# YXHXianYu/RVCP-Real-Time-Path-Tracer

Measured on AMD Instinct MI355X. Metric: Msamples/sec (pixels*SPP/s) + frame ms, Cornell Box 1024^2 SPP=30, higher is better.
Workload: dtype f32

## Files before the change

### rvcp-real-time-path-tracer_amd/csrc/embed_src.py

```python
#!/usr/bin/env python3
import hashlib
import sys

NAMES = ["kJitSrcKernels", "kJitSrcInternal", "kJitSrcAbi", "kJitSrcSqrt", "kJitSrcTonemap"]
DELIM = "RVCPSRC"


def build_id(out, srcs):
    h = hashlib.sha256()
    for path in srcs:
        data = open(path, "rb").read()
        h.update(path.encode() + b"\0" + str(len(data)).encode() + b"\0" + data)
    with open(out, "w") as f:
        f.write("// generated by embed_src.py --build-id; do not edit\n#pragma once\n"
                f'static const char kRvcpSourceHash[] = "{h.hexdigest()[:16]}";\n')


def main():
    if sys.argv[1] == "--build-id":
        return build_id(sys.argv[2], sys.argv[3:])
    out, srcs = sys.argv[1], sys.argv[2:]
    parts = ["// generated by embed_src.py from " + " ".join(srcs) + "; do not edit", "#pragma once"]
    for name, path in zip(NAMES, srcs):
        text = open(path).read()
        assert ")" + DELIM + '"' not in text
        parts.append(f'static const char {name}[] = R"{DELIM}(' + text + f'){DELIM}";')
    with open(out, "w") as f:
        f.write("\n".join(parts) + "\n")


if __name__ == "__main__":
    main()
```

### rvcp-real-time-path-tracer_amd/csrc/rvcp_jit.cpp

```cpp
#include <hip/hip_runtime.h>

#include <dlfcn.h>
#include <sys/stat.h>
#include <unistd.h>

#include <algorithm>
#include <atomic>
#include <cerrno>
#include <cmath>
#include <cstdint>
#include <cstdio>
#include <cstdlib>
#include <cstring>
#include <list>
#include <memory>
#include <mutex>
#include <map>
#include <string>
#include <vector>

#include "rvcp_internal.h"
#include "rvcp_jit.h"
#include "build/rvcp_jit_src.h"

// ... 789 lines not shown
    e = std::getenv("RVCP_DEBUG_SPEC_EAGER");
    if (e && *e == '1') opts |= kScanEagerSplit;
#endif
    return opts;
}

std::vector<std::string> jit_options(const JitCompile &cc);

std::string jit_sampling_tag(int sampling)
{
    return sampling == RVCP_SAMPLING_UNIFORM ? std::string()
                                             : "// +sampling " + std::to_string(sampling) + "\n";
}

std::string jit_spp_map_tag(bool spp_map)
{
    return spp_map ? std::string("// +spp_map\n") : std::string();
}

namespace {

uint64_t fnv1a(const std::string &s)
{
    uint64_t h = 1469598103934665603ull;
    for (unsigned char c : s) {
        h ^= c;
        h *= 1099511628211ull;
    }
    return h;
}

struct CacheEntry {
    int device;
    uint64_t hash;
    std::string scan;
    std::shared_ptr<JitKernels> kernels;
};
std::mutex g_mu;
std::list<CacheEntry> g_cache;
constexpr size_t kCacheEntries = 16;

constexpr char kCoMagic[8] = {'R', 'V', 'C', 'P', 'C', 'O', '0', '1'};
std::string g_cache_dir;
bool g_cache_dir_set = false;
std::atomic<uint64_t> g_disk_loads{0}, g_disk_compiles{0}, g_disk_rejects{0};

std::string default_cache_dir()
{
    const char *x = std::getenv("XDG_CACHE_HOME");
    if (x && *x == '/') return std::string(x) + "/rvcp-mi355x";
    const char *h = std::getenv("HOME");
    if (h && *h == '/') return std::string(h) + "/.cache/rvcp-mi355x";
    return std::string();
}

std::string cache_dir()
{
    if (!g_cache_dir_set) {
        g_cache_dir = default_cache_dir();
        g_cache_dir_set = true;
    }
    return g_cache_dir;
}

bool make_dirs(const std::string &dir)
{
    if (dir.empty()) return false;
    for (size_t i = 1; i <= dir.size(); i++) {
        if (i == dir.size() || dir[i] == '/') {
            const std::string p = dir.substr(0, i);
            if (::mkdir(p.c_str(), 0700) != 0 && errno != EEXIST) return false;
        }
    }
    struct stat st;
    return ::stat(dir.c_str(), &st) == 0 && S_ISDIR(st.st_mode);
}

std::string code_key(const std::string &scan, const std::vector<std::string> &opts)
{
    int maj = -1, mnr = -1;
    if (rtc().version) (void)rtc().version(&maj, &mnr);
    std::string k = "rvcp code object\nhiprtc " + std::to_string(maj) + "." + std::to_string(mnr) + "\n";
    for (const std::string &o : opts) k += o + "\n";
    for (const char *src : {kJitSrcKernels, kJitSrcInternal, kJitSrcAbi, kJitSrcSqrt, kJitSrcTonemap}) {
        const std::string s(src);
        k += "src " + std::to_string(s.size()) + " " + std::to_string(fnv1a(s)) + "\n";
    }
    return k + scan;
}

std::string hex64(uint64_t v)
{
    char b[17];
    std::snprintf(b, sizeof(b), "%016llx", (unsigned long long)v);
    return b;
}

uint64_t fnv1a_bytes(const char *p, size_t n)
{
    uint64_t h = 1469598103934665603ull;
    for (size_t i = 0; i < n; i++) {
        h ^= (unsigned char)p[i];
        h *= 1099511628211ull;
    }
    return h;
}

int disk_read(const std::string &dir, const std::string &key, std::vector<char> &code)
{
    const std::string path = dir + "/" + hex64(fnv1a(key)) + ".rvcpco";
    std::FILE *f = std::fopen(path.c_str(), "rb");
    if (!f) return 0;
    std::vector<char> buf;
    char tmp[1 << 16];
    size_t got;
    while ((got = std::fread(tmp, 1, sizeof(tmp), f)) > 0) buf.insert(buf.end(), tmp, tmp + got);
    std::fclose(f);
    uint64_t hdr[4];
    if (buf.size() < 8 + sizeof(hdr) || std::memcmp(buf.data(), kCoMagic, 8) != 0) return -1;
    std::memcpy(hdr, buf.data() + 8, sizeof(hdr));
    const size_t off = 8 + sizeof(hdr);
    if (hdr[0] != key.size() || hdr[1] == 0 || buf.size() - off < hdr[0] ||
        buf.size() - off - hdr[0] != hdr[1] ||
        hdr[3] != fnv1a(key) || std::memcmp(buf.data() + off, key.data(), key.size()) != 0)
        return -1;
    const char *c = buf.data() + off + hdr[0];
    if (fnv1a_bytes(c, hdr[1]) != hdr[2] || hdr[1] < 4 || std::memcmp(c, "\x7f" "ELF", 4) != 0)
        return -1;
    code.assign(c, c + hdr[1]);
    return 1;
}

void disk_write(const std::string &dir, const std::string &key, const std::vector<char> &code)
{
    if (!make_dirs(dir)) return;
    static std::atomic<unsigned> seq{0};
    const std::string path = dir + "/" + hex64(fnv1a(key)) + ".rvcpco";
    const std::string tmp = path + ".tmp." + std::to_string((long)::getpid()) + "." + std::to_string(seq++);
    std::FILE *f = std::fopen(tmp.c_str(), "wb");
    if (!f) return;
    const uint64_t hdr[4] = {key.size(), code.size(), fnv1a_bytes(code.data(), code.size()), fnv1a(key)};
    bool ok = std::fwrite(kCoMagic, 1, 8, f) == 8 && std::fwrite(hdr, 1, sizeof(hdr), f) == sizeof(hdr) &&
              std::fwrite(key.data(), 1, key.size(), f) == key.size() &&
              std::fwrite(code.data(), 1, code.size(), f) == code.size();
    ok = (std::fclose(f) == 0) && ok;
    if (!ok || std::rename(tmp.c_str(), path.c_str()) != 0) std::remove(tmp.c_str());
}

}

int jit_cached_code(const std::string &scan, std::vector<char> &code, std::string &err,
                    const JitCompile &cc, bool *from_disk, bool force_compile)
{
    *from_disk = false;
    const std::string dir = cache_dir();
    std::string key;
    if (!dir.empty()) {
        key = code_key(scan, jit_options(cc));
        if (force_compile) {
            g_disk_rejects++;
        } else {
            const int r = disk_read(dir, key, code);
            if (r == 1) {
                g_disk_loads++;
                *from_disk = true;
                return 0;
            }
            if (r < 0) g_disk_rejects++;
        }
    }
    if (jit_compile_code(scan, code, err, cc) != 0) return -1;
    g_disk_compiles++;
    if (!dir.empty()) disk_write(dir, key, code);
    return 0;
}

JitKernels::~JitKernels()
{
    if (module) {
        int cur = -1;
        (void)hipGetDevice(&cur);
        (void)hipSetDevice(device);
        (void)hipModuleUnload(module);
        if (cur >= 0) (void)hipSetDevice(cur);
    }
}

std::vector<std::string> jit_options(const JitCompile &cc)
{
    std::vector<std::string> opts = {"--offload-arch=gfx950", "-O3", "-std=c++17",
                                     "-ffp-contract=off", "-fhip-fp32-correctly-rounded-divide-sqrt",
                                     "-fno-fast-math", "-fno-slp-vectorize", "-DRVCP_JIT",
                                     "-DRVCP_SPEC_SCAN=\"rvcp_spec_scan.inc\""};
    if (cc.legacy) opts.push_back("-DRVCP_JIT_LEGACY");
    if (cc.bvh) opts.push_back("-DRVCP_JIT_BVH");
    if (cc.sampling != RVCP_SAMPLING_UNIFORM)
        opts.push_back("-DRVCP_SAMPLING=" + std::to_string(cc.sampling));
    if (cc.spp_map) opts.push_back("-DRVCP_SPP_MAP=1");
#ifdef RVCP_TIMELINE
    opts.push_back("-DRVCP_TIMELINE");
#endif
    if (cc.legacy && cc.legacy_waves > 0)
        opts.push_back("-DRVCP_LEGACY_MIN_WAVES=" + std::to_string(cc.legacy_waves));
    if (cc.legacy && cc.lds_scene) opts.push_back("-DRVCP_LEGACY_LDS_SCENE");
    for (const std::string &x : jit_extra_flags()) opts.push_back(x);
    return opts;
}

int jit_compile_code(const std::string &scan, std::vector<char> &code, std::string &err,
                     const JitCompile &cc)
{
    const RtcApi &api = rtc();
    if (!api.ok) {
        err = api.why;
        return -1;
    }
    const char *hdr_src[] = {kJitSrcInternal, kJitSrcAbi, kJitSrcSqrt, kJitSrcTonemap, scan.c_str()};
    const char *hdr_name[] = {"rvcp_internal.h", "../../include/rvcp.h", "rvcp_sqrt.h", "rvcp_tonemap.h",
                              "rvcp_spec_scan.inc"};
    rtc_program prog = nullptr;
    if (api.create(&prog, kJitSrcKernels, "rvcp_kernels.hip", 5, hdr_src, hdr_name) != 0) {
        err = "hiprtcCreateProgram failed";
        return -1;
    }
    const std::vector<std::string> opt_s = jit_options(cc);
    std::vector<const char *> opts;
    for (const std::string &x : opt_s) opts.push_back(x.c_str());
    const int rc = api.compile(prog, (int)opts.size(), opts.data());
    if (rc != 0) {
        size_t ls = 0;
        api.log_size(prog, &ls);
        std::string log(ls, '\0');
        if (ls) api.log(prog, &log[0]);
        err = "hipRTC compile failed: " + log.substr(0, 4000);
        api.destroy(&prog);
        return -1;
    }
    size_t cs = 0;
    api.code_size(prog, &cs);
    code.assign(cs, 0);
    if (cs) api.code(prog, code.data());
    api.destroy(&prog);
    return cs ? 0 : -1;
}

std::string jit_module_source(const TriRecord *tri, uint32_t n, const JitSpec &spec, JitCompile &cc)
{
    cc = JitCompile{};
    cc.legacy = spec.legacy;
    cc.lds_scene = spec.legacy && spec.lds_fits;
#ifndef RVCP_SPHERELESS_LEGACY_WAVES
#define RVCP_SPHERELESS_LEGACY_WAVES 6
#endif
    cc.legacy_waves = spec.legacy && spec.sphereless ? RVCP_SPHERELESS_LEGACY_WAVES : cc.lds_scene ? 5 : 0;
#ifdef RVCP_DEBUG_KNOBS
    if (const char *e = std::getenv("RVCP_JIT_LEGACY_WAVES")) cc.legacy_waves = std::atoi(e);
#endif
    cc.bvh = spec.bvh;
    cc.sampling = spec.sampling;
    cc.spp_map = spec.spp_map;
    std::string key_flags;
    for (const std::string &x : jit_extra_flags()) key_flags += " " + x;
    return jit_scan_source(tri, n, jit_scan_opts()) +
        (spec.legacy || spec.bvh ? std::string() : jit_groups_source(tri, n, spec.lum_mask, jit_scan_opts())) +
        (spec.legacy ? "// +legacy " + std::to_string(cc.legacy_waves) + (cc.lds_scene ? " lds" : "") + "\n"
#ifndef RVCP_NO_SPHERE_LITERALS
                      + jit_sphere_source(spec.spheres, spec.n_spheres)
#endif
                      + (cc.lds_scene ? jit_legacy_lds_source(n, spec.n_spheres, spec.n_materials) : std::string())
                : std::string()) +
        (key_flags.empty() ? std::string() : "// +flags" + key_flags + "\n") +
        (spec.bvh ? "// +bvh\n" : "") +
        jit_sampling_tag(spec.sampling) + jit_spp_map_tag(spec.spp_map);
}

std::shared_ptr<JitKernels> jit_path_kernels(int device, const TriRecord *tri, uint32_t n,
                                             const JitSpec &spec, std::string &err)
{
    JitCompile cc;
    const std::string scan = jit_module_source(tri, n, spec, cc);
    const bool legacy = spec.legacy, bvh = spec.bvh;
    const uint64_t h = fnv1a(scan);
    std::lock_guard<std::mutex> lock(g_mu);
    for (auto it = g_cache.begin(); it != g_cache.end(); ++it) {
        if (it->device == device && it->hash == h && it->scan == scan) {
            g_cache.splice(g_cache.begin(), g_cache, it);
            return g_cache.front().kernels;
        }
    }
    if (hipSetDevice(device) != hipSuccess) {
        err = "hipSetDevice failed";
        return nullptr;
    }
    auto load = [&](JitKernels &k, const std::vector<char> &code) -> std::string {
        if (hipModuleLoadData(&k.module, code.data()) != hipSuccess) {
            k.module = nullptr;
            return "hipModuleLoadData failed";
        }
        if (hipModuleGetFunction(&k.path5, k.module, "rvcp_spec_path_kernel5") != hipSuccess ||
            hipModuleGetFunction(&k.path6, k.module, "rvcp_spec_path_kernel6") != hipSuccess)
            return "specialised kernels missing from the module";
        if (hipModuleGetFunction(&k.primary, k.module, "rvcp_spec_primary_kernel") != hipSuccess)
            return "specialised pre-pass kernel missing from the module";
        if (bvh && (hipModuleGetFunction(&k.bvh_path, k.module, "rvcp_spec_bvh_path_kernel") != hipSuccess ||
// ... 283 lines not shown
```

### rvcp-real-time-path-tracer_amd/csrc/rvcp_kernels.hip

```cpp
#ifndef __HIPCC_RTC__
#include <hip/hip_runtime.h>
#endif

#ifndef RVCP_SAMPLING
#define RVCP_SAMPLING 0
#endif
#ifndef RVCP_SPP_MAP
#define RVCP_SPP_MAP 0
#endif
#if RVCP_SPP_MAP
#define RVCP_SPP_MAP_PARAM , const uint32_t *__restrict__ spp_map
#define RVCP_SPP_MAP_ARG , spp_map
#else
#define RVCP_SPP_MAP_PARAM
#define RVCP_SPP_MAP_ARG
#endif
#define RVCP_GAMES101_ONLY (RVCP_SAMPLING || RVCP_SPP_MAP)

#include "rvcp_internal.h"
#include "../../include/rvcp.h"
#include "rvcp_sqrt.h"
#include "rvcp_tonemap.h"

#if defined(RVCP_JIT) || !RVCP_GAMES101_ONLY
#define RVCP_BUILD_TAG
#elif RVCP_SAMPLING && RVCP_SPP_MAP
#define RVCP_BUILD_TAG cosine_map_
#elif RVCP_SPP_MAP
#define RVCP_BUILD_TAG map_
#else
#define RVCP_BUILD_TAG cosine_
#endif
#define RVCP_PASTE3_(a, b, c) a##b##c
#define RVCP_PASTE3(a, b, c) RVCP_PASTE3_(a, b, c)
#define RVCP_G101(name) RVCP_PASTE3(games101_, RVCP_BUILD_TAG, name)
#define RVCP_KERNEL_BUILD RVCP_PASTE3(rvcp_games101_, RVCP_BUILD_TAG, build)
#if RVCP_SPP_MAP
#define RVCP_G101_PRIMARY RVCP_G101(primary_kernel)
#else
#define RVCP_G101_PRIMARY games101_primary_kernel
#endif

namespace rvcp {
namespace {

struct f3 { float x, y, z; };
__device__ __forceinline__ f3 mk(float x, float y, float z) { return f3{x, y, z}; }
__device__ __forceinline__ f3 add(f3 a, f3 b) { return mk(a.x + b.x, a.y + b.y, a.z + b.z); }
__device__ __forceinline__ f3 sub(f3 a, f3 b) { return mk(a.x - b.x, a.y - b.y, a.z - b.z); }
__device__ __forceinline__ f3 mulv(f3 a, f3 b) { return mk(a.x * b.x, a.y * b.y, a.z * b.z); }
__device__ __forceinline__ f3 muls(f3 a, float s) { return mk(a.x * s, a.y * s, a.z * s); }
__device__ __forceinline__ f3 divs(f3 a, float s) { return mk(a.x / s, a.y / s, a.z / s); }
__device__ __forceinline__ f3 neg(f3 a) { return mk(-a.x, -a.y, -a.z); }
__device__ __forceinline__ float dot(f3 a, f3 b) {
    return __builtin_fmaf(a.z, b.z, __builtin_fmaf(a.y, b.y, a.x * b.x));
}
__device__ __forceinline__ f3 cross(f3 a, f3 b) {
    return mk(__builtin_fmaf(a.y, b.z, -(a.z * b.y)), __builtin_fmaf(a.z, b.x, -(a.x * b.z)),
              __builtin_fmaf(a.x, b.y, -(a.y * b.x)));
}
__device__ __forceinline__ float sqrt_c(float x) { return sqrt_ieee(x); }
__device__ __forceinline__ float len(f3 a) { return sqrt_c(dot(a, a)); }
__device__ __forceinline__ float rcp_ieee(float den);
__device__ __forceinline__ f3 normalize(f3 a) {
    const float x = dot(a, a);
    const float s = sqrt_fast_core(x);
    const float y = __builtin_amdgcn_rcpf(s);
    float r = __builtin_fmaf(__builtin_fmaf(-s, y, 1.0f), y, y);
    if (__builtin_expect(!sqrt_fast_ok(x), 0)) r = rcp_ieee(__builtin_sqrtf(x));
    return muls(a, r);
}
__device__ __forceinline__ float fractf(float x) { return x - __builtin_floorf(x); }
__device__ __forceinline__ f3 ld3(const float *p) { return mk(p[0], p[1], p[2]); }

constexpr uint32_t kLight = 3u;

constexpr float kInvPi = 0x1.45f306p-2f;
constexpr float kPiHi = 0x1.921fb6p+1f;
constexpr float kPiLo = 0x1.777a5cp-24f;
__device__ __forceinline__ float sin_poly(float r) {
    const float z = r * r;
    const float p = __builtin_fmaf(__builtin_fmaf(__builtin_fmaf(0x1.5dbdfep-19f, z, -0x1.9f7p-13f),
                                                  z, 0x1.110ed4p-7f), z, -0x1.55554cp-3f);
    return __builtin_fmaf(p, z * r, r);
}
__device__ __forceinline__ float pt_sinf(float x) {
    if (!(__builtin_fabsf(x) < 1.0e30f)) return x - x;
    const float q = __builtin_rintf(x * kInvPi);
    float r = __builtin_fmaf(q, -kPiHi, x);
    r = __builtin_fmaf(q, kPiLo, r);
    const float s = sin_poly(r);
    const float odd = q - 2.0f * __builtin_floorf(q * 0.5f);
    return odd != 0.0f ? -s : s;
}

__device__ __forceinline__ float pt_sinf_rand(float x) {
    const float q = __builtin_rintf(x * kInvPi);
    float r = __builtin_fmaf(q, -kPiHi, x);
    r = __builtin_fmaf(q, kPiLo, r);
    const float s = sin_poly(r);
    return __uint_as_float(__float_as_uint(s) + ((uint32_t)(int)q << 31));
}

__device__ __forceinline__ uint32_t lane_id() {
    return __builtin_amdgcn_mbcnt_hi(~0u, __builtin_amdgcn_mbcnt_lo(~0u, 0u));
// ... 65 lines not shown
    if (A.want_linear) {
        out_lin[3 * (size_t)pix + 0] = acc.x;
        out_lin[3 * (size_t)pix + 1] = acc.y;
        out_lin[3 * (size_t)pix + 2] = acc.z;
    }
}

__device__ __forceinline__ void store_acc(uint32_t pix, f3 acc, float *__restrict__ lin) {
    lin[3 * (size_t)pix + 0] = acc.x;
    lin[3 * (size_t)pix + 1] = acc.y;
    lin[3 * (size_t)pix + 2] = acc.z;
}

struct TriPart {
    f3 s2;
    float den, n1, n2;
};
__device__ __forceinline__ TriPart tri_stage1(const TriRecord &T, f3 o, f3 d) {
    const f3 s = mk(o.x - T.v0[0], o.y - T.v0[1], o.z - T.v0[2]);
    const f3 e1 = ld3(T.e1);
    const f3 s1 = cross(d, ld3(T.e2));
    TriPart P;
    P.s2 = cross(s, e1);
    P.den = dot(s1, e1);
    P.n1 = dot(s1, s);
    P.n2 = dot(P.s2, d);
    return P;
}
__device__ __forceinline__ float rcp_scan_fast(float den);
template <bool FAST = false>
__device__ __forceinline__ bool tri_stage2(const TriRecord &T, const TriPart &P, float tmin,
                                           float bt, float &t_out) {
    const float f = FAST ? rcp_scan_fast(P.den) : rcp_scan(P.den);
    const float t = f * dot(P.s2, ld3(T.e2));
    const float b1 = f * P.n1;
    const float b2 = f * P.n2;
    t_out = t;
    return (b1 >= 0.0f) & (b2 >= 0.0f) & (b1 + b2 <= 1.0f) & (t >= tmin) & (t <= bt);
}
template <bool FAST = false>
__device__ __forceinline__ bool tri_accept(const TriRecord &T, f3 o, f3 d, float tmin, float bt,
                                           float &t_out) {
    return tri_stage2<FAST>(T, tri_stage1(T, o, d), tmin, bt, t_out);
}
__device__ __forceinline__ float rcp_scan_fast(float den) {
    const float r = __builtin_amdgcn_rcpf(den);
    return __builtin_fmaf(__builtin_fmaf(-den, r, 1.0f), r, r);
}
__device__ __forceinline__ bool dir_grain_ok(f3 d) {
    const uint32_t x = (__float_as_uint(d.x) << 1) - 1u, y = (__float_as_uint(d.y) << 1) - 1u,
                   z = (__float_as_uint(d.z) << 1) - 1u;
    return min(min(x, y), z) >= (0x2B800000u << 1) - 1u;
}
__device__ __forceinline__ bool dir_fast_ok(f3 d) {
    return (((__builtin_fabsf(d.x) + __builtin_fabsf(d.y)) + __builtin_fabsf(d.z)) <= 16.0f) &
           dir_grain_ok(d);
}
#ifdef RVCP_SPEC_SCAN
#define RVCP_F32(bits) __uint_as_float(bits)
#define RVCP_SPEC_COMMIT(t, i) do { asm volatile("" : "+v"(t), "+v"(i)); \
                                    __builtin_amdgcn_sched_barrier(0); } while (0)
#define RVCP_SPEC_COMMIT1(t) do { asm volatile("" : "+v"(t)); \
                                  __builtin_amdgcn_sched_barrier(0); } while (0)
#ifdef RVCP_SPEC_NO_SKIP
#define RVCP_SPEC_ANY(q) ((void)(q), true)
#elif defined(RVCP_SPEC_ISA_SKIP_ALL)
#define RVCP_SPEC_ANY(q) ((void)(q), false)
#else
#define RVCP_SPEC_ANY(q) (__builtin_amdgcn_ballot_w64(q) != 0ull)
#endif
#define RVCP_SPEC_RCP(den) rcp_scan(den)
#define RVCP_SPEC_RCP_FAST(den) rcp_scan_fast(den)
#define RVCP_SPEC_BOX_RCP(x) __builtin_amdgcn_rcpf(x)
#include RVCP_SPEC_SCAN
__device__ __forceinline__ bool ray_in_range(f3 o, f3 d) {
    return (((__builtin_fabsf(o.x) + __builtin_fabsf(o.y)) + __builtin_fabsf(o.z)) <= 0x1p41f) &
           (((__builtin_fabsf(d.x) + __builtin_fabsf(d.y)) + __builtin_fabsf(d.z)) <= 16.0f) &
           dir_grain_ok(d);
}
#ifdef RVCP_SPEC_GROUPS
__device__ __forceinline__ bool spec_ray_ok(f3 o, f3 d) {
    return ray_in_range(o, d) & spec_group_origin_ok(o);
}
__device__ __forceinline__ void spec_group_pass(float4 *rows, float tmin, bool hasA, f3 a_o, f3 a_d,
                                                float &btA, bool hasB, f3 b_o, f3 b_d, float &btB,
                                                int &bestB) {
    const uint32_t rA = hasA ? spec_group_reach(a_o, a_d, tmin, btA) : 0u;
    const uint32_t rB = hasB ? spec_group_reach(b_o, b_d, tmin, btB) : 0u;
    if (__builtin_amdgcn_ballot_w64((rA | rB) != 0u) == 0ull) return;
    uint64_t m[2 * RVCP_SPEC_GROUPS];
    uint32_t base[2 * RVCP_SPEC_GROUPS], total = 0u;
#pragma unroll
    for (int g = 0; g < RVCP_SPEC_GROUPS; g++) {
        m[2 * g] = __builtin_amdgcn_ballot_w64(((rA >> g) & 1u) != 0u);
        base[2 * g] = total;
        total += (uint32_t)__builtin_popcountll(m[2 * g]);
        m[2 * g + 1] = __builtin_amdgcn_ballot_w64(((rB >> g) & 1u) != 0u);
        base[2 * g + 1] = total;
        total += (uint32_t)__builtin_popcountll(m[2 * g + 1]);
    }
    for (uint32_t p0 = 0u; p0 < total; p0 += (uint32_t)kWave) {
        __builtin_amdgcn_fence(__ATOMIC_RELEASE, "wavefront");
        __builtin_amdgcn_wave_barrier();
        __builtin_amdgcn_fence(__ATOMIC_ACQUIRE, "wavefront");
#pragma unroll
        for (int g = 0; g < RVCP_SPEC_GROUPS; g++) {
            const uint32_t jA = base[2 * g] + rank_in(m[2 * g]) - p0;
            if (((rA >> g) & 1u) != 0u && jA < (uint32_t)kWave) {
                rows[2 * jA] = make_float4(a_o.x, a_o.y, a_o.z, btA);
                rows[2 * jA + 1] = make_float4(a_d.x, a_d.y, a_d.z, __int_as_float(g));
            }
            const uint32_t jB = base[2 * g + 1] + rank_in(m[2 * g + 1]) - p0;
            if (((rB >> g) & 1u) != 0u && jB < (uint32_t)kWave) {
                rows[2 * jB] = make_float4(b_o.x, b_o.y, b_o.z, btB);
                rows[2 * jB + 1] = make_float4(b_d.x, b_d.y, b_d.z, __int_as_float(g));
            }
        }
        __builtin_amdgcn_fence(__ATOMIC_RELEASE, "wavefront");
        __builtin_amdgcn_wave_barrier();
        __builtin_amdgcn_fence(__ATOMIC_ACQUIRE, "wavefront");
        const uint32_t lane_r = lane_id();
        const float4 ro = rows[2 * lane_r], rd = rows[2 * lane_r + 1];
        float bt = ro.w;
        int best = -1;
        if (lane_r < total - p0)
            spec_group_scan(__float_as_int(rd.w), mk(ro.x, ro.y, ro.z), mk(rd.x, rd.y, rd.z), tmin, bt, best);
        __builtin_amdgcn_fence(__ATOMIC_RELEASE, "wavefront");
        __builtin_amdgcn_wave_barrier();
        __builtin_amdgcn_fence(__ATOMIC_ACQUIRE, "wavefront");
        rows[2 * lane_r] = make_float4(bt, __int_as_float(best), 0.0f, 0.0f);
        __builtin_amdgcn_fence(__ATOMIC_RELEASE, "wavefront");
        __builtin_amdgcn_wave_barrier();
        __builtin_amdgcn_fence(__ATOMIC_ACQUIRE, "wavefront");
#pragma unroll
        for (int g = 0; g < RVCP_SPEC_GROUPS; g++) {
            const uint32_t jA = base[2 * g] + rank_in(m[2 * g]) - p0;
            if (((rA >> g) & 1u) != 0u && jA < (uint32_t)kWave) {
                const float4 r = rows[2 * jA];
                if (__float_as_int(r.y) >= 0 && r.x < btA) btA = r.x;
            }
            const uint32_t jB = base[2 * g + 1] + rank_in(m[2 * g + 1]) - p0;
            if (((rB >> g) & 1u) != 0u && jB < (uint32_t)kWave) {
                const float4 r = rows[2 * jB];
                const int ob = __float_as_int(r.y);
                if (ob >= 0 && (r.x < btB || (r.x == btB && ob > bestB))) { btB = r.x; bestB = ob; }
            }
        }
    }
}
#endif
#endif
struct TriPartA {
    f3 s, s1;
    float den, n1, m;
};
__device__ __forceinline__ TriPartA tri_stage1a(const TriRecord &T, f3 o, f3 d) {
    TriPartA P;
    P.s = mk(o.x - T.v0[0], o.y - T.v0[1], o.z - T.v0[2]);
    P.s1 = cross(d, ld3(T.e2));
    P.den = dot(P.s1, ld3(T.e1));
    P.n1 = dot(P.s1, P.s);
    P.m = __builtin_fabsf(P.den) * 1.00000095367431640625f;
    return P;
}
__device__ __forceinline__ bool tri_maybe_a(const TriPartA &P) { return __builtin_fabsf(P.n1) <= P.m; }
__device__ __forceinline__ TriPart tri_stage1b(const TriRecord &T, const TriPartA &Pa, f3 d) {
    TriPart P;
    P.s2 = cross(Pa.s, ld3(T.e1));
    P.den = Pa.den;
    P.n1 = Pa.n1;
    P.n2 = dot(P.s2, d);
    return P;
}
__device__ __forceinline__ bool tri_maybe(const TriPart &P) {
    const float m = __builtin_fabsf(P.den) * 1.00000095367431640625f;
    return (__builtin_fabsf(P.n1) <= m) & (__builtin_fabsf(P.n2) <= m);
}

__device__ __forceinline__ bool slab(const float *b, f3 o, f3 inv, float tmin, float bt,
                                     float &tnear) {
    const float x0 = (b[0] - o.x) * inv.x, x1 = (b[3] - o.x) * inv.x;
    const float y0 = (b[1] - o.y) * inv.y, y1 = (b[4] - o.y) * inv.y;
    const float z0 = (b[2] - o.z) * inv.z, z1 = (b[5] - o.z) * inv.z;
    const float tn = __builtin_fmaxf(__builtin_fmaxf(__builtin_fminf(x0, x1), __builtin_fminf(y0, y1)),
                                     __builtin_fmaxf(__builtin_fminf(z0, z1), tmin));
    const float tf = __builtin_fminf(__builtin_fminf(__builtin_fmaxf(x0, x1), __builtin_fmaxf(y0, y1)),
                                     __builtin_fminf(__builtin_fmaxf(z0, z1), bt));
    tnear = tn;
    return tn <= tf;
}

constexpr uint32_t kBvhLeafChunk = 4;
template <uint32_t kCh = kBvhLeafChunk>
__device__ __forceinline__ void bvh_leaf(const TriRecord *__restrict__ btri, int32_t ref, f3 o, f3 d,
                                         float tmin, float &bt, int &best, uint32_t slots = 0) {
    const uint32_t code = ~(uint32_t)ref;
    const uint32_t first = code >> 5, cnt = (code & 31u) + 1u;
    for (uint32_t c0 = 0; c0 < cnt; c0 += kCh) {
        const float4 *base = reinterpret_cast<const float4 *>(
            reinterpret_cast<const float *>(btri + slots) + 10u * (first + c0));
        const uint32_t nc = cnt - c0 < kCh ? cnt - c0 : kCh;
        const uint32_t nld = (10u * nc + 3u) >> 2;
        float4 W[(10 * kCh + 3) / 4];
#pragma unroll
        for (uint32_t k = 0; k < (uint32_t)((10 * kCh + 3) / 4); ++k)
            if (k < nld) W[k] = base[k];
        const float *F = reinterpret_cast<const float *>(W);
#pragma unroll
        for (uint32_t k = 0; k < kCh; ++k) {
            if (k < nc) {
                TriRecord T;
#pragma unroll
                for (int c = 0; c < 3; ++c) {
                    T.v0[c] = F[10 * k + c];
                    T.e1[c] = F[10 * k + 3 + c];
                    T.e2[c] = F[10 * k + 6 + c];
                }
                float t;
                const int id = __float_as_int(F[10 * k + 9]);
                if (tri_accept(T, o, d, tmin, bt, t) && (t < bt || id > best)) {
                    bt = t;
                    best = id;
                }
            }
        }
// ... 2036 lines not shown
                         newA ? shadow_stop(A.eps, A.t_min, a_p, nee_dist) : -__builtin_inff());
#endif
            } else
            {
            if (A.bvh_prefix)
                bvh_prefix_scan<false>(A, tri, sA, sB, s_ao, s_ad, b_o, b_d, btA, bestA, btB, bestB);
            if (sA) bvh_nearest<true>(bvh_nodes, bvh_tris, A.bvh_root, stk, s_ao, s_ad, A.t_min, btA, bestA, A.bvh_n4, A.bvh_slots);
            if (sB) bvh_nearest<true>(bvh_nodes, bvh_tris, A.bvh_root, stk, b_o, b_d, A.t_min, btB, bestB, A.bvh_n4, A.bvh_slots);
            }
        } else if (tail) {
            uint32_t R = 2;
            while (nr * R * 2 <= (uint32_t)kWave) R *= 2;
            uint8_t *tab = tail_tab[wv];
            if (hasA) tab[rank_in(mA)] = (uint8_t)lane;
            if (hasB) tab[na + rank_in(mB)] = (uint8_t)lane;
            __builtin_amdgcn_fence(__ATOMIC_RELEASE, "wavefront");
            __builtin_amdgcn_wave_barrier();
            __builtin_amdgcn_fence(__ATOMIC_ACQUIRE, "wavefront");
            const uint32_t j = lane / R, part = lane % R;
            const bool worker = j < nr;
            const int owner = worker ? (int)tab[j] : (int)lane;
            const bool isA = j < na;
            f3 o, d;
            {
                const f3 oa = mk(__shfl(a_o.x, owner), __shfl(a_o.y, owner), __shfl(a_o.z, owner));
                const f3 da = mk(__shfl(a_d.x, owner), __shfl(a_d.y, owner), __shfl(a_d.z, owner));
                const f3 ob = mk(__shfl(b_o.x, owner), __shfl(b_o.y, owner), __shfl(b_o.z, owner));
                const f3 db = mk(__shfl(b_d.x, owner), __shfl(b_d.y, owner), __shfl(b_d.z, owner));
                o = isA ? oa : ob;
                d = isA ? da : db;
            }
            float bt = A.t_max;
            int best = -1;
            if (worker) {
                if (A.rcp_fast && !__any(worker && !dir_fast_ok(d))) {
                    for (uint32_t i = part; i < A.n_faces; i += R) {
                        float t;
                        if (tri_accept<true>(tri[i], o, d, A.t_min, bt, t)) { bt = t; best = (int)i; }
                    }
                } else {
                    for (uint32_t i = part; i < A.n_faces; i += R) {
                        float t;
                        if (tri_accept(tri[i], o, d, A.t_min, bt, t)) { bt = t; best = (int)i; }
                    }
                }
            }
            for (uint32_t off = R >> 1; off >= 1; off >>= 1) {
                const float ot = __shfl_xor(bt, (int)off);
                const int ob = __shfl_xor(best, (int)off);
                if (ot < bt || (ot == bt && ob > best)) { bt = ot; best = ob; }
            }
            const int srcA = hasA ? (int)(rank_in(mA) * R) : (int)lane;
            const int srcB = hasB ? (int)((na + rank_in(mB)) * R) : (int)lane;
            const float tA_ = __shfl(bt, srcA), tB_ = __shfl(bt, srcB);
            const int iA_ = __shfl(best, srcA), iB_ = __shfl(best, srcB);
            if (hasA) { btA = tA_; bestA = iA_; }
            if (hasB) { btB = tB_; bestB = iB_; }
        } else if (!TILED && wave_active && nr <= (uint32_t)kWave) {
            float4 *rows = compact_lds + wv * (2 * kWave);
            if (hasA) {
                const uint32_t j = rank_in(mA);
                rows[2 * j] = make_float4(a_o.x, a_o.y, a_o.z, 0.0f);
                rows[2 * j + 1] = make_float4(a_d.x, a_d.y, a_d.z, 0.0f);
            }
            if (hasB) {
                const uint32_t j = na + rank_in(mB);
                rows[2 * j] = make_float4(b_o.x, b_o.y, b_o.z, 0.0f);
                rows[2 * j + 1] = make_float4(b_d.x, b_d.y, b_d.z, 0.0f);
            }
            __builtin_amdgcn_fence(__ATOMIC_RELEASE, "wavefront");
            __builtin_amdgcn_wave_barrier();
            __builtin_amdgcn_fence(__ATOMIC_ACQUIRE, "wavefront");
            uint32_t lane_r;
            asm volatile("v_mbcnt_lo_u32_b32 %0, -1, 0\n\tv_mbcnt_hi_u32_b32 %0, -1, %0"
                         : "=v"(lane_r));
            const float4 ro = rows[2 * lane_r], rd = rows[2 * lane_r + 1];
            const f3 o = mk(ro.x, ro.y, ro.z), d = mk(rd.x, rd.y, rd.z);
            float bt = A.t_max;
            int best = -1;
#ifdef RVCP_SPEC_GROUPS
            if (!__any(lane_r < nr && !spec_ray_ok(o, d))) {
                spec_always1(o, d, A.t_min, bt, best);
                float no_bt = -1.0f;
                spec_group_pass(rows, A.t_min, false, o, d, no_bt, lane_r < nr, o, d, bt, best);
            } else
#elif defined(RVCP_SPEC_SCAN)
            if (!__any(lane_r < nr && !ray_in_range(o, d))) {
                spec_scan1(o, d, A.t_min, bt, best);
            } else
#endif
            if (A.rcp_fast && !__any(lane_r < nr && !dir_fast_ok(d)))
                scan_generic1<true>(tri, A.n_faces, o, d, A.t_min, bt, best);
            else
                scan_generic1<false>(tri, A.n_faces, o, d, A.t_min, bt, best);
            __builtin_amdgcn_fence(__ATOMIC_RELEASE, "wavefront");
            __builtin_amdgcn_wave_barrier();
            __builtin_amdgcn_fence(__ATOMIC_ACQUIRE, "wavefront");
            rows[2 * lane_r] = make_float4(bt, __int_as_float(best), 0.0f, 0.0f);
            __builtin_amdgcn_fence(__ATOMIC_RELEASE, "wavefront");
            __builtin_amdgcn_wave_barrier();
            __builtin_amdgcn_fence(__ATOMIC_ACQUIRE, "wavefront");
            if (hasA) {
                const float4 r = rows[2 * rank_in(mA)];
                btA = r.x;
                bestA = __float_as_int(r.y);
            }
            if (hasB) {
                const float4 r = rows[2 * (na + rank_in(mB))];
                btB = r.x;
                bestB = __float_as_int(r.y);
            }
        } else {
#ifdef RVCP_SPEC_GROUPS
            if (!TILED && !BVH &&
                !__any((hasA && !spec_ray_ok(a_o, a_d)) || (hasB && !spec_ray_ok(b_o, b_d)))) {
                if (!hasA) btA = -1.0f;
                spec_always2(a_o, a_d, b_o, b_d, A.t_min, btA, btB, bestB);
                spec_group_pass(compact_lds + wv * (2 * kWave), A.t_min, hasA, a_o, a_d, btA, hasB,
                                b_o, b_d, btB, bestB);
            } else
#elif defined(RVCP_SPEC_SCAN)
            if (!__any((hasA && !ray_in_range(a_o, a_d)) || (hasB && !ray_in_range(b_o, b_d)))) {
                if (!hasA) btA = -1.0f;
                spec_scan2(a_o, a_d, b_o, b_d, A.t_min, btA, btB, bestB);
            } else
#endif
            {
            if (!SINGLE && !hasA) btA = -1.0f;
            if (A.rcp_fast && !__any((hasA && !dir_fast_ok(a_d)) || (hasB && !dir_fast_ok(b_d))))
                scan_generic2<true, SINGLE>(tri, A.n_faces, a_o, a_d, b_o, b_d, A.t_min, btA, bestA, btB, bestB);
            else
                scan_generic2<false, SINGLE>(tri, A.n_faces, a_o, a_d, b_o, b_d, A.t_min, btA, bestA, btB, bestB);
            }
            if (!SINGLE) {
                bestA = btA != A.t_max ? 0 : -1;
                if (__builtin_expect(__any(hasA && btA == A.t_max), 0)) {
                    btA = A.t_max;
                    bestA = -1;
                    for (uint32_t i = 0; i < A.n_faces; ++i) {
                        float tA;
                        if (tri_accept(tri[i], a_o, a_d, A.t_min, btA, tA)) { btA = tA; bestA = (int)i; }
                    }
                }
            }
        }

        if (SINGLE && !hasA) {
            btB = btA;
            bestB = bestA;
        }
        RC_END(1);
        RC_BEGIN(3);

        if (LDS_STATE) col = st_get3(13);
        if (hasA && !frozen) {
            if (LDS_STATE) {
                a_p = st_get3(0);
                nee_C = st_get3(3);
                nee_dist = st[6 * BLK];
            }
            const f3 hp = bestA >= 0 ? add(a_o, muls(a_d, btA))
                                     : mk(__builtin_inff(), __builtin_inff(), __builtin_inff());
            const float dist_blocked = len(sub(hp, a_p));
            if (__builtin_fabsf(nee_dist - dist_blocked) < A.eps) {
                col = add(col, nee_C);
                if (LDS_STATE) st_put3(13, col);
            }
        }
        const bool defer_B = SINGLE && hasA && hasB;
        if (frozen) {
        } else if (hasB && !defer_B) {
            if (bestB < 0) {
                col = add(col, mk(0.1f, 0.1f, 0.1f));
                if (LDS_STATE) st_put3(13, col);
                ended = true;
            } else {
                f3 hpos, hn;
                FaceShade fs;
                hit_shade(tri, shade, bestB, b_o, b_d, btB, hpos, hn, fs);
                if (fs.ty == kLight) {
                    ended = true;
                } else {
                    S_pos = hpos; S_nrm = hn; S_alb = ld3(fs.alb_pi);
                    surf_ev = true;
                }
            }
        } else if (hasA && !hasB) {
            ended = true;
        }
        if (!frozen) {
            hasA = false;
            if (!defer_B) hasB = false;
        }
        RC_END(3);
#ifdef RVCP_REGION_CLOCK
        c_iter += __builtin_amdgcn_s_memtime() - c_top;
#endif
    }
    flush_wave_counters(counters, lane, trav_wave, iters);
    clock_stamp(counters, lane, wv == 0, true);
#ifdef RVCP_TIMELINE
    if (A.timeline && lane == 0) {
// ... 1273 lines not shown
```

Before: 11820.

## Pack spec group work so each group scan fits within one wave pass

Replaces the contiguous packing of per-group ray work in spec_group_pass with a packer that aligns a group to a 64-lane pass boundary whenever it would otherwise straddle two passes. The aim is that each group's triangles are scanned in fewer passes, so lanes do less split work across passes. Per-lane slot indices are precomputed into packed bytes, and groups that are not in the current pass are skipped. In exchange it can add passes through padding, adds bookkeeping per pass, and includes optional RVCP_GROUP_COUNT instrumentation.

```diff
diff --git a/rvcp-real-time-path-tracer_amd/csrc/embed_src.py b/rvcp-real-time-path-tracer_amd/csrc/embed_src.py
--- a/rvcp-real-time-path-tracer_amd/csrc/embed_src.py
+++ b/rvcp-real-time-path-tracer_amd/csrc/embed_src.py
@@ -2,7 +2,7 @@
 import hashlib
 import sys
 
-NAMES = ["kJitSrcKernels", "kJitSrcInternal", "kJitSrcAbi", "kJitSrcSqrt", "kJitSrcTonemap"]
+NAMES = ["kJitSrcKernels", "kJitSrcInternal", "kJitSrcAbi", "kJitSrcSqrt", "kJitSrcTonemap", "kJitSrcGroupPack"]
 DELIM = "RVCPSRC"
 
 
diff --git a/rvcp-real-time-path-tracer_amd/csrc/rvcp_group_pack.h b/rvcp-real-time-path-tracer_amd/csrc/rvcp_group_pack.h
--- /dev/null
+++ b/rvcp-real-time-path-tracer_amd/csrc/rvcp_group_pack.h
@@ -0,0 +1,53 @@
+#pragma once
+#ifndef __HIPCC_RTC__
+#include <stdint.h>
+#endif
+
+#if defined(__HIPCC__) || defined(__HIPCC_RTC__)
+#define RVCP_GROUP_PACK_FN __host__ __device__ __forceinline__
+#else
+#define RVCP_GROUP_PACK_FN static inline
+#endif
+
+#define RVCP_GROUP_PACK_MAX_GROUPS 4
+#define RVCP_GROUP_PACK_WIDTH 64u
+
+RVCP_GROUP_PACK_FN uint32_t rvcp_group_pack(const uint32_t *c, int n_groups, uint32_t *start) {
+    uint32_t f = 0u;
+    for (int g = 0; g < n_groups; g++) {
+#ifndef RVCP_GROUP_PACK_CONTIGUOUS
+        if (c[g] != 0u && (f & 63u) + ((c[g] - 1u) & 63u) + 1u > RVCP_GROUP_PACK_WIDTH)
+            f = (f + 63u) & ~63u;
+#endif
+        start[g] = f;
+        f += c[g];
+    }
+    return (f + 63u) >> 6;
+}
+
+RVCP_GROUP_PACK_FN bool rvcp_group_pack_in_pass(uint32_t c_g, uint32_t start_g, uint32_t p) {
+    return c_g != 0u && start_g < 64u * p + 64u && start_g + c_g > 64u * p;
+}
+
+RVCP_GROUP_PACK_FN void rvcp_group_pack_span(uint32_t c_g, uint32_t start_g, uint32_t p, uint32_t *lo,
+                                             uint32_t *hi) {
+    const uint32_t p0 = 64u * p, e = start_g + c_g;
+    *lo = start_g > p0 ? start_g - p0 : 0u;
+    *hi = e < p0 + 64u ? e - p0 : 64u;
+}
+
+RVCP_GROUP_PACK_FN uint32_t rvcp_group_pack_lanes(const uint32_t *c, const uint32_t *start, int n_groups,
+                                                  uint32_t p) {
+    uint32_t n = 0u;
+    for (int g = 0; g < n_groups; g++)
+        if (rvcp_group_pack_in_pass(c[g], start[g], p)) {
+            uint32_t lo, hi;
+            rvcp_group_pack_span(c[g], start[g], p, &lo, &hi);
+            if (hi > n) n = hi;
+        }
+    return n;
+}
+
+RVCP_GROUP_PACK_FN uint32_t rvcp_group_pack_item(uint32_t start_g, uint32_t n_a, int slot_b, uint32_t rank) {
+    return start_g + (slot_b ? n_a : 0u) + rank;
+}
diff --git a/rvcp-real-time-path-tracer_amd/csrc/rvcp_jit.cpp b/rvcp-real-time-path-tracer_amd/csrc/rvcp_jit.cpp
--- a/rvcp-real-time-path-tracer_amd/csrc/rvcp_jit.cpp
+++ b/rvcp-real-time-path-tracer_amd/csrc/rvcp_jit.cpp
@@ -895,7 +895,7 @@
     if (rtc().version) (void)rtc().version(&maj, &mnr);
     std::string k = "rvcp code object\nhiprtc " + std::to_string(maj) + "." + std::to_string(mnr) + "\n";
     for (const std::string &o : opts) k += o + "\n";
-    for (const char *src : {kJitSrcKernels, kJitSrcInternal, kJitSrcAbi, kJitSrcSqrt, kJitSrcTonemap}) {
+    for (const char *src : {kJitSrcKernels, kJitSrcInternal, kJitSrcAbi, kJitSrcSqrt, kJitSrcTonemap, kJitSrcGroupPack}) {
         const std::string s(src);
         k += "src " + std::to_string(s.size()) + " " + std::to_string(fnv1a(s)) + "\n";
     }
@@ -1028,11 +1028,12 @@
         err = api.why;
         return -1;
     }
-    const char *hdr_src[] = {kJitSrcInternal, kJitSrcAbi, kJitSrcSqrt, kJitSrcTonemap, scan.c_str()};
+    const char *hdr_src[] = {kJitSrcInternal, kJitSrcAbi, kJitSrcSqrt, kJitSrcTonemap, kJitSrcGroupPack,
+                             scan.c_str()};
     const char *hdr_name[] = {"rvcp_internal.h", "../../include/rvcp.h", "rvcp_sqrt.h", "rvcp_tonemap.h",
-                              "rvcp_spec_scan.inc"};
+                              "rvcp_group_pack.h", "rvcp_spec_scan.inc"};
     rtc_program prog = nullptr;
-    if (api.create(&prog, kJitSrcKernels, "rvcp_kernels.hip", 5, hdr_src, hdr_name) != 0) {
+    if (api.create(&prog, kJitSrcKernels, "rvcp_kernels.hip", 6, hdr_src, hdr_name) != 0) {
         err = "hiprtcCreateProgram failed";
         return -1;
     }
diff --git a/rvcp-real-time-path-tracer_amd/csrc/rvcp_kernels.hip b/rvcp-real-time-path-tracer_amd/csrc/rvcp_kernels.hip
--- a/rvcp-real-time-path-tracer_amd/csrc/rvcp_kernels.hip
+++ b/rvcp-real-time-path-tracer_amd/csrc/rvcp_kernels.hip
@@ -21,6 +21,7 @@
 #include "../../include/rvcp.h"
 #include "rvcp_sqrt.h"
 #include "rvcp_tonemap.h"
+#include "rvcp_group_pack.h"
 
 #if defined(RVCP_JIT) || !RVCP_GAMES101_ONLY
 #define RVCP_BUILD_TAG
@@ -252,36 +253,58 @@
 __device__ __forceinline__ bool spec_ray_ok(f3 o, f3 d) {
     return ray_in_range(o, d) & spec_group_origin_ok(o);
 }
+#ifdef RVCP_GROUP_COUNT
+#define RVCP_GC_PARAMS , unsigned long long &gc_sum, unsigned long long &gc_n
+#define RVCP_GC_ARGS , c_scan, c_iter
+#else
+#define RVCP_GC_PARAMS
+#define RVCP_GC_ARGS
+#endif
 __device__ __forceinline__ void spec_group_pass(float4 *rows, float tmin, bool hasA, f3 a_o, f3 a_d,
                                                 float &btA, bool hasB, f3 b_o, f3 b_d, float &btB,
-                                                int &bestB) {
+                                                int &bestB RVCP_GC_PARAMS) {
     const uint32_t rA = hasA ? spec_group_reach(a_o, a_d, tmin, btA) : 0u;
     const uint32_t rB = hasB ? spec_group_reach(b_o, b_d, tmin, btB) : 0u;
     if (__builtin_amdgcn_ballot_w64((rA | rB) != 0u) == 0ull) return;
-    uint64_t m[2 * RVCP_SPEC_GROUPS];
-    uint32_t base[2 * RVCP_SPEC_GROUPS], total = 0u;
+    uint32_t cnt[RVCP_SPEC_GROUPS], start[RVCP_SPEC_GROUPS], iA = 0u, iB = 0u;
 #pragma unroll
     for (int g = 0; g < RVCP_SPEC_GROUPS; g++) {
-        m[2 * g] = __builtin_amdgcn_ballot_w64(((rA >> g) & 1u) != 0u);
-        base[2 * g] = total;
-        total += (uint32_t)__builtin_popcountll(m[2 * g]);
-        m[2 * g + 1] = __builtin_amdgcn_ballot_w64(((rB >> g) & 1u) != 0u);
-        base[2 * g + 1] = total;
-        total += (uint32_t)__builtin_popcountll(m[2 * g + 1]);
-    }
-    for (uint32_t p0 = 0u; p0 < total; p0 += (uint32_t)kWave) {
+        const uint64_t mA = __builtin_amdgcn_ballot_w64(((rA >> g) & 1u) != 0u);
+        const uint64_t mB = __builtin_amdgcn_ballot_w64(((rB >> g) & 1u) != 0u);
+        const uint32_t nA = (uint32_t)__builtin_popcountll(mA);
+        cnt[g] = nA + (uint32_t)__builtin_popcountll(mB);
+        if (((rA >> g) & 1u) != 0u) iA |= (0x80u | rvcp_group_pack_item(0u, nA, 0, rank_in(mA))) << (8 * g);
+        if (((rB >> g) & 1u) != 0u) iB |= (0x80u | rvcp_group_pack_item(0u, nA, 1, rank_in(mB))) << (8 * g);
+    }
+    const uint32_t passes = rvcp_group_pack(cnt, RVCP_SPEC_GROUPS, start);
+#ifdef RVCP_GROUP_COUNT
+    {
+        uint32_t total = 0u, scans = 0u;
+        for (int g = 0; g < RVCP_SPEC_GROUPS; g++) {
+            total += cnt[g];
+            for (uint32_t p = 0u; p < passes; p++) scans += rvcp_group_pack_in_pass(cnt[g], start[g], p) ? 1u : 0u;
+        }
+        gc_sum += RVCP_GROUP_COUNT == 1 ? total : RVCP_GROUP_COUNT == 2 ? passes
+                : RVCP_GROUP_COUNT == 3 ? scans : (total > 64u ? 1u : 0u);
+        gc_n += 1ull;
+    }
+#endif
+    for (uint32_t p = 0u; p < passes; p++) {
+        const uint32_t p0 = p * (uint32_t)kWave;
         __builtin_amdgcn_fence(__ATOMIC_RELEASE, "wavefront");
         __builtin_amdgcn_wave_barrier();
         __builtin_amdgcn_fence(__ATOMIC_ACQUIRE, "wavefront");
 #pragma unroll
         for (int g = 0; g < RVCP_SPEC_GROUPS; g++) {
-            const uint32_t jA = base[2 * g] + rank_in(m[2 * g]) - p0;
-            if (((rA >> g) & 1u) != 0u && jA < (uint32_t)kWave) {
+            if (!rvcp_group_pack_in_pass(cnt[g], start[g], p)) continue;
+            const uint32_t eA = (iA >> (8 * g)) & 0xFFu, eB = (iB >> (8 * g)) & 0xFFu;
+            const uint32_t jA = (eA & 0x7Fu) + (start[g] - p0);
+            if ((eA & 0x80u) != 0u && jA < (uint32_t)kWave) {
                 rows[2 * jA] = make_float4(a_o.x, a_o.y, a_o.z, btA);
                 rows[2 * jA + 1] = make_float4(a_d.x, a_d.y, a_d.z, __int_as_float(g));
             }
-            const uint32_t jB = base[2 * g + 1] + rank_in(m[2 * g + 1]) - p0;
-            if (((rB >> g) & 1u) != 0u && jB < (uint32_t)kWave) {
+            const uint32_t jB = (eB & 0x7Fu) + (start[g] - p0);
+            if ((eB & 0x80u) != 0u && jB < (uint32_t)kWave) {
                 rows[2 * jB] = make_float4(b_o.x, b_o.y, b_o.z, btB);
                 rows[2 * jB + 1] = make_float4(b_d.x, b_d.y, b_d.z, __int_as_float(g));
             }
@@ -293,7 +316,7 @@
         const float4 ro = rows[2 * lane_r], rd = rows[2 * lane_r + 1];
         float bt = ro.w;
         int best = -1;
-        if (lane_r < total - p0)
+        if (lane_r < rvcp_group_pack_lanes(cnt, start, RVCP_SPEC_GROUPS, p))
             spec_group_scan(__float_as_int(rd.w), mk(ro.x, ro.y, ro.z), mk(rd.x, rd.y, rd.z), tmin, bt, best);
         __builtin_amdgcn_fence(__ATOMIC_RELEASE, "wavefront");
         __builtin_amdgcn_wave_barrier();
@@ -304,13 +327,15 @@
         __builtin_amdgcn_fence(__ATOMIC_ACQUIRE, "wavefront");
 #pragma unroll
         for (int g = 0; g < RVCP_SPEC_GROUPS; g++) {
-            const uint32_t jA = base[2 * g] + rank_in(m[2 * g]) - p0;
-            if (((rA >> g) & 1u) != 0u && jA < (uint32_t)kWave) {
+            if (!rvcp_group_pack_in_pass(cnt[g], start[g], p)) continue;
+            const uint32_t eA = (iA >> (8 * g)) & 0xFFu, eB = (iB >> (8 * g)) & 0xFFu;
+            const uint32_t jA = (eA & 0x7Fu) + (start[g] - p0);
+            if ((eA & 0x80u) != 0u && jA < (uint32_t)kWave) {
                 const float4 r = rows[2 * jA];
                 if (__float_as_int(r.y) >= 0 && r.x < btA) btA = r.x;
             }
-            const uint32_t jB = base[2 * g + 1] + rank_in(m[2 * g + 1]) - p0;
-            if (((rB >> g) & 1u) != 0u && jB < (uint32_t)kWave) {
+            const uint32_t jB = (eB & 0x7Fu) + (start[g] - p0);
+            if ((eB & 0x80u) != 0u && jB < (uint32_t)kWave) {
                 const float4 r = rows[2 * jB];
                 const int ob = __float_as_int(r.y);
                 if (ob >= 0 && (r.x < btB || (r.x == btB && ob > bestB))) { btB = r.x; bestB = ob; }
@@ -2513,7 +2538,7 @@
             if (!__any(lane_r < nr && !spec_ray_ok(o, d))) {
                 spec_always1(o, d, A.t_min, bt, best);
                 float no_bt = -1.0f;
-                spec_group_pass(rows, A.t_min, false, o, d, no_bt, lane_r < nr, o, d, bt, best);
+                spec_group_pass(rows, A.t_min, false, o, d, no_bt, lane_r < nr, o, d, bt, best RVCP_GC_ARGS);
             } else
 #elif defined(RVCP_SPEC_SCAN)
             if (!__any(lane_r < nr && !ray_in_range(o, d))) {
@@ -2548,7 +2573,7 @@
                 if (!hasA) btA = -1.0f;
                 spec_always2(a_o, a_d, b_o, b_d, A.t_min, btA, btB, bestB);
                 spec_group_pass(compact_lds + wv * (2 * kWave), A.t_min, hasA, a_o, a_d, btA, hasB,
-                                b_o, b_d, btB, bestB);
+                                b_o, b_d, btB, bestB RVCP_GC_ARGS);
             } else
 #elif defined(RVCP_SPEC_SCAN)
             if (!__any((hasA && !ray_in_range(a_o, a_d)) || (hasB && !ray_in_range(b_o, b_d)))) {
```

After: 12430 (median of 6 runs). 5.2% higher.
